# opherlieber/rltime

Measured on AMD Instinct MI355X. Metric: sampled transitions/sec (= learner steps/sec x B x T), IQN-LSTM B=512 T=80 84x84x4, higher is better.
Workload: dtype f32

## Files before the change

### include/mirl.h

```cpp
#ifndef MIRL_H
#define MIRL_H

#include <stdint.h>

#ifdef __cplusplus
extern "C" {
#endif

#define MIRL_OK 0
#define MIRL_NEED_MORE 1
#define MIRL_ERR_ARG (-1)
#define MIRL_ERR_HIP (-2)
#define MIRL_ERR_STATE (-3)
#define MIRL_ERR_NOGPU (-4)

#define MIRL_MODE_UNIFORM 0
#define MIRL_MODE_PER 1

typedef struct mirl_replay mirl_replay;

typedef struct mirl_replay_config {
  int64_t size;
  int32_t num_envs;
  int32_t env_base;
// ... 202 lines not shown
                              float* db, void* stream);

int mirl_conv1p3_u8_supported(int32_t H, int32_t W, int32_t F, int32_t K, int32_t S);
int mirl_conv1p3_u8_wpk_floats(int64_t* out);
int mirl_conv1p3_u8_fwd(int64_t N, int32_t H, int32_t W, const uint8_t* x, const float* weight,
                        int64_t ws_o, int64_t ws_c, int64_t ws_h, int64_t ws_w, const float* bias, float scale,
                        float* wpk, float* y, int32_t flags, void* stream);
int mirl_conv1p3_u8_wrw_scratch_floats(int64_t* out);
int mirl_conv1p3_u8_wrw(int64_t N, int32_t H, int32_t W, const uint8_t* x, const float* g, float scale,
                        float* scratch, float* dw, int64_t ws_o, int64_t ws_c, int64_t ws_h, int64_t ws_w, void* stream);
int mirl_conv1p3_u8_wrw_masked(int64_t N, int32_t H, int32_t W, const uint8_t* x, const float* dy, const float* y,
                               float scale, float* scratch, float* dw, int64_t ws_o, int64_t ws_c, int64_t ws_h,
                               int64_t ws_w, float* db, void* stream);

int mirl_conv2_bwd_data_supported(int32_t C, int32_t F, int32_t K, int32_t S, int32_t IH, int32_t IW,
                                  int32_t OH, int32_t OW);
int mirl_conv2_bwd_data(int64_t N, int32_t OH, int32_t OW, const float* g, const float* weight,
                        int64_t ws_o, int64_t ws_c, int64_t ws_h, int64_t ws_w, float* wpk, float* dx,
                        void* stream);
int mirl_conv2_bwd_data_wpk_floats(int64_t* floats);
int mirl_conv2_bwd_data_ex(int64_t N, int32_t OH, int32_t OW, const float* g, const float* weight, int64_t ws_o,
                           int64_t ws_c, int64_t ws_h, int64_t ws_w, float* wpk, int64_t wpk_floats, float* dx, int32_t pipe,
                           void* stream);
int mirl_conv3_bwd_data_supported(int32_t C, int32_t F, int32_t K, int32_t S, int32_t IH, int32_t IW, int32_t OH, int32_t OW);
int mirl_conv3_bwd_data_wpk_floats(int64_t* floats);
int mirl_conv3_bwd_data(int64_t N, int32_t OH, int32_t OW, const float* g, const float* weight, int64_t ws_o,
                        int64_t ws_c, int64_t ws_h, int64_t ws_w, float* wpk, int64_t wpk_floats, float* dx, void* stream);

int mirl_gemm3_supported(int32_t layout, int64_t M, int64_t N, int64_t K);
int mirl_gemm3_workspace_bytes(int32_t layout, int64_t M, int64_t N, int64_t K, int64_t* bytes);
int mirl_gemm3(int32_t layout, int64_t M, int64_t N, int64_t K, const float* A, int64_t lda,
               const float* B, int64_t ldb, float* C, int64_t ldc, const float* bias, int32_t relu,
               void* workspace, int64_t workspace_bytes, void* stream);
int mirl_gemm3_mid_set(int32_t mode);
int mirl_gemm3_nt_mul(int64_t M, int64_t N, int64_t K, const float* A, int64_t lda, const float* B,
                      int64_t ldb, float* C, int64_t ldc, const float* bias, int32_t relu,
                      const float* mul, int64_t ldmul, int32_t group_shift, float* pre, int64_t ldpre,
                      void* stream);
int mirl_gemm3_head_workspace_bytes(int64_t M, int64_t N, int64_t* bytes);
int mirl_gemm3_nt_head(int64_t M, int64_t N, int64_t K, const float* A, int64_t lda, const float* B, int64_t ldb,
                       float* C, int64_t ldc, const float* bias, int32_t relu, const float* w2, int32_t O,
                       const float* bias2, float* out2, int64_t ldo, void* workspace, int64_t workspace_bytes, void* stream);
int mirl_gemm3_nn_qp_partial_rows(int64_t M, int64_t* rows);
int mirl_gemm3_nn_qp(int64_t M, int64_t N, int64_t K, const float* A, int64_t lda, const float* B, int64_t ldb,
                     const float* emb, int64_t ldemb, const float* x, int64_t ldx, float* d_pre, int64_t ldd,
                     float* dx, int64_t lddx, float* db_partial, void* stream);

int mirl_conv3_fwd_supported(int32_t C, int32_t F, int32_t KH, int32_t KW, int32_t S, int32_t H, int32_t W);
int mirl_conv3_fwd(int64_t N, int32_t H, int32_t W, int32_t C, int32_t F, int32_t KH, int32_t KW, int32_t S,
                   const float* x, const float* w, const float* bias, int32_t relu, float* y, void* stream);

int mirl_conv_wrw_b3_supported(int32_t C, int32_t F, int32_t KH, int32_t KW, int32_t S, int32_t H, int32_t W);
int mirl_conv_wrw_b3_scratch_bytes(int32_t C, int32_t F, int32_t KH, int32_t KW, int64_t* bytes);
int mirl_conv_wrw_b3(int64_t N, int32_t H, int32_t W, int32_t C, int32_t F, int32_t KH, int32_t KW, int32_t S,
                     const float* x, const float* g, void* scratch, int64_t scratch_bytes, float* dw, void* stream);

int mirl_bias_relu_rows(int64_t rows, int32_t C, float* y, const float* bias, void* stream);
int mirl_colsum_blocks(int64_t rows, int32_t C, int32_t* blocks);
int mirl_relu_bwd_bias_rows(int64_t rows, int32_t C, const float* dy, const float* y, float* g,
                            float* db, float* partial, int32_t blocks, void* stream);
int mirl_cos_embed(int64_t rows, int32_t D, const float* tau, const float* freq, float* phi, void* stream);
int mirl_cos_embed_rng(int64_t rows, int32_t D, uint64_t seed, const uint64_t* step, const float* freq,
                       float* phi, float* tau_out, void* stream);
int mirl_iqn_mul_fwd(int64_t M, int32_t N, int32_t C, const float* x, const float* emb, float* out, void* stream);
int mirl_iqn_mul_bwd(int64_t M, int32_t N, int32_t C, const float* g, const float* emb, const float* x,
                     float* d_pre, float* dx, float* db, float* partial, int32_t blocks, void* stream);

int mirl_dueling_tail_bwd(int64_t M, int32_t H1, int32_t Hv, int32_t A, int32_t Q, const float* ga,
                          const float* gv, const float* wo, const float* wq, const float* both,
                          float* g, float* db, float* partial, int32_t blocks, void* stream);
int mirl_dueling_tail_bwd_w(int64_t M, int32_t H1, int32_t Hv, int32_t A, int32_t Q, const float* ga,
                            const float* gv, const float* wo, const float* wq, const float* both, float* g,
                            float* db, float* partial, int32_t blocks, float* dwj, float* partial_w,
                            void* stream);

int mirl_actor_head(int32_t E, int32_t N, int32_t A, const float* adv, const float* val, int32_t Q,
                    const double* eps, const double* expo, double eps_min, const float* u, const int64_t* rnd,
                    int32_t* actions, float* qvalues, float* eps_used, void* stream);
int mirl_actor_head_rng(int32_t E, int32_t N, int32_t A, const float* adv, int32_t adv_pitch, const float* val, int32_t Q,
                        const double* eps, const double* expo, double eps_min, uint64_t rng_seed,
                        const uint64_t* rng_step, int32_t* actions, float* qvalues, float* eps_used, void* stream);
int mirl_actor_head_c51(int32_t E, int32_t A, int32_t Z, const float* adv, int32_t adv_pitch, const float* val,
                        int32_t val_pitch, const float* support, const double* eps, const double* expo, double eps_min,
                        const float* u, const int64_t* rnd, uint64_t rng_seed, const uint64_t* rng_step,
                        int32_t* actions, float* qvalues, float* eps_used, void* stream);
int mirl_stack_shift(int32_t E, int32_t P, int32_t plane_bytes, const uint8_t* in, uint8_t* out,
                     const uint8_t* newest, const uint8_t* dones, void* stream);
#define MIRL_STEP_ADVANCE (~0ull)
int mirl_actor_pre(int32_t E, int32_t H, int32_t A, const float* rewards_raw, const uint8_t* dones,
                   const int32_t* actions, const float* h, const float* c, float* xh_tail, int64_t xh_pitch,
                   float* c_in, float* state_pack, float* initials, float* rewards_out, uint8_t* dones_out,
                   int32_t clip_rewards, float* ep_reward, int32_t* ep_len, float* out_reward, int32_t* out_len,
                   int32_t* action_counts, uint64_t* rng_step, uint64_t step, void* stream);
int mirl_synth_env_step(int32_t E, int64_t frame_bytes, const uint8_t* pool, int32_t pool_n, uint64_t* clock, int32_t slot,
                        uint64_t seed, float p_neg, float p_nonpos, float p_done, uint8_t* obs, float* rewards,
                        uint8_t* dones, void* stream);
int mirl_act_conv_supported(int32_t layer, int32_t Ci, int32_t Co, int32_t k, int32_t stride, int32_t Hi, int32_t Wi);
int mirl_act_conv_fwd(int32_t layer, int64_t frames, int32_t Hi, int32_t Wi, const float* x, const float* w_taps,
                      const float* bias, float* y, int64_t y_frame_pitch, void* stream);
int mirl_act_lstm_supported(int32_t E, int32_t H, int32_t K);
int mirl_act_lstm_workspace_bytes(int32_t E, int32_t H, int32_t K, int64_t* bytes);
int mirl_act_lstm_fwd(int32_t E, int32_t H, int32_t K, const float* xh, int64_t xh_pitch, const float* w, const float* bias,
                      const float* c_in, float* h_out, float* c_out, void* workspace, void* stream);
int mirl_act_embed(int32_t E, int32_t N, int32_t H, int32_t D, const float* h, const float* freq, const float* taus,
                   uint64_t seed, const uint64_t* step, const float* wq, const float* bq, float* x, float* tau_out, void* stream);
int mirl_act_head_supported(int32_t E, int32_t N, int32_t H, int32_t D, int32_t HID, int32_t NO);
// ... 153 lines not shown
```

### rltime_amd/_lib.py

```python
import ctypes as C
import os

import torch

_HERE = os.path.dirname(os.path.abspath(__file__))
LIB_PATH = os.path.join(_HERE, "librltime_hip.so")

MIRL_OK = 0
MIRL_NEED_MORE = 1
MODE_UNIFORM = 0
MODE_PER = 1
INT32_MIN = -2 ** 31


MIRL_OK, MIRL_ERR_ARG, MIRL_ERR_HIP, MIRL_ERR_STATE, MIRL_ERR_NOGPU = 0, -1, -2, -3, -4


class MirlError(RuntimeError):
    code = None


class ReplayConfig(C.Structure):
    _fields_ = [
        ("size", C.c_int64),
# ... 118 lines not shown
    "mirl_q_target_c51": [_i64, _i32, _i32, _vp, _vp, _vp, _vp, _vp, _vp, _f64, _f64, _f64, _f64, _i32, _vp, _vp],
    "mirl_loss_c51": [_i64, _i32, _i32, _vp, _vp, _vp, _vp, _i32, _f64, _f64, _vp, _vp, _vp, _vp],
    "mirl_actor_head_c51": [_i32, _i32, _i32, _vp, _i32, _vp, _i32, _vp, _vp, _vp, _f64, _vp, _vp, _u64, _vp, _vp, _vp, _vp, _vp],
    "mirl_lstm_cell_fwd": [_i32, _i32, _vp, _vp, _vp, _vp, _vp, _vp, _vp, _vp],
    "mirl_lstm_seq_supported": [_i32, _i32, _i32],
    "mirl_lstm_seq_workspace_bytes": [_i32, _i32, _P(_i64)],
    "mirl_lstm_seq_fwd": [_i32, _i32, _i32, _vp, _vp, _vp, _vp, _vp, _vp, _vp, _vp, _vp, _vp, _vp, _i32, _vp, _vp],
    "mirl_lstm_seq_status": [_P(_i32)],
    "mirl_gemm3_mid_set": [_i32],
    "mirl_lstm_seq_fwd_grid": [_i32, _i32, _P(_i32), _P(_i64), _P(_i32), _P(_i32)],
    "mirl_lstm_seq_bwd_supported": [_i32, _i32, _i32],
    "mirl_lstm_seq_bwd_workspace_bytes": [_i32, _i32, _P(_i64)],
    "mirl_lstm_seq_bwd": [_i32, _i32, _i32, _vp, _vp, _vp, _vp, _vp, _vp, _vp, _vp],
    "mirl_lstm_cell_bwd": [_i32, _i32, _vp, _vp, _vp, _vp, _vp, _vp, _vp, _i32, _vp],
    "mirl_lstm_extras_supported": [_i64, _i64, _i32],
    "mirl_lstm_extras_add": [_i64, _i64, _i32, _vp, _i64, _vp, _i64, _vp, _i64, _vp, _i64, _vp],
    "mirl_lstm_extras_wgrad_workspace_bytes": [_i64, _i64, _i32, _P(_i64)],
    "mirl_lstm_extras_wgrad": [_i64, _i64, _i32, _vp, _i64, _vp, _i64, _vp, _vp, _i64, _vp],
    "mirl_frames_to_f32_nhwc": [_i64, _i32, _i32, _vp, C.c_float, _vp, _vp],
    "mirl_frames_to_f32_nhwc_ex": [_i64, _i32, _i32, _vp, C.c_float, _vp, _i32, _i32, _vp],
    "mirl_conv1_u8_supported": [_i32, _i32, _i32, _i32, _i32, _i32],
    "mirl_conv1_bf16_set": [_i32],
    "mirl_conv1_wrw_bf16_set": [_i32],
    "mirl_conv1_u8_wpk_floats": [_P(_i64)],
    "mirl_conv1_u8_fwd": [_i64, _i32, _i32, _vp, _vp, _i64, _i64, _i64, _i64, _vp, C.c_float, _vp, _vp, _vp],
    "mirl_conv1_u8_fwd_ex": [_i64, _i32, _i32, _vp, _vp, _i64, _i64, _i64, _i64, _vp, C.c_float, _vp, _vp, _i32, _vp],
    "mirl_conv1_u8_wrw_scratch_floats": [_P(_i64)],
    "mirl_conv1_u8_wrw_ex": [_i64, _i32, _i32, _vp, _vp, C.c_float, _vp, _vp, _i64, _i64, _i64, _i64, _i32, _vp],
    "mirl_conv1_u8_wrw_masked": [_i64, _i32, _i32, _vp, _vp, _vp, C.c_float, _vp, _vp, _i64, _i64, _i64, _i64, _vp, _vp],
    "mirl_conv1_u8_wrw": [_i64, _i32, _i32, _vp, _vp, C.c_float, _vp, _vp, _i64, _i64, _i64, _i64, _vp],
    "mirl_conv1p_u8_supported": [_i32, _i32, _i32, _i32, _i32],
    "mirl_conv1p_u8_wpk_floats": [_P(_i64)],
    "mirl_conv1p_u8_fwd": [_i64, _i32, _i32, _vp, _vp, _i64, _i64, _i64, _vp, C.c_float, _vp, _vp, _i32, _vp],
    "mirl_conv1p_u8_wrw_scratch_floats": [_P(_i64)],
    "mirl_conv1p_u8_wrw": [_i64, _i32, _i32, _vp, _vp, C.c_float, _vp, _vp, _i64, _i64, _i64, _vp],
    "mirl_conv1p_u8_wrw_masked": [_i64, _i32, _i32, _vp, _vp, _vp, C.c_float, _vp, _vp, _i64, _i64, _i64, _vp, _vp],
    "mirl_conv1p3_u8_supported": [_i32, _i32, _i32, _i32, _i32],
    "mirl_conv1p3_u8_wpk_floats": [_P(_i64)],
    "mirl_conv1p3_u8_fwd": [_i64, _i32, _i32, _vp, _vp, _i64, _i64, _i64, _i64, _vp, C.c_float, _vp, _vp, _i32, _vp],
    "mirl_conv1p3_u8_wrw_scratch_floats": [_P(_i64)],
    "mirl_conv1p3_u8_wrw": [_i64, _i32, _i32, _vp, _vp, C.c_float, _vp, _vp, _i64, _i64, _i64, _i64, _vp],
    "mirl_conv1p3_u8_wrw_masked": [_i64, _i32, _i32, _vp, _vp, _vp, C.c_float, _vp, _vp, _i64, _i64, _i64, _i64, _vp, _vp],
    "mirl_conv2_bwd_data_supported": [_i32, _i32, _i32, _i32, _i32, _i32, _i32, _i32],
    "mirl_conv2_bwd_data": [_i64, _i32, _i32, _vp, _vp, _i64, _i64, _i64, _i64, _vp, _vp, _vp],
    "mirl_conv2_bwd_data_wpk_floats": [_P(_i64)],
    "mirl_conv3_bwd_data_supported": [_i32, _i32, _i32, _i32, _i32, _i32, _i32, _i32],
    "mirl_conv3_bwd_data_wpk_floats": [_P(_i64)],
    "mirl_conv3_bwd_data": [_i64, _i32, _i32, _vp, _vp, _i64, _i64, _i64, _i64, _vp, _i64, _vp, _vp],
    "mirl_conv2_bwd_data_ex": [_i64, _i32, _i32, _vp, _vp, _i64, _i64, _i64, _i64, _vp, _i64, _vp, _i32, _vp],
    "mirl_conv3_fwd_supported": [_i32, _i32, _i32, _i32, _i32, _i32, _i32],
    "mirl_conv3_fwd": [_i64, _i32, _i32, _i32, _i32, _i32, _i32, _i32, _vp, _vp, _vp, _i32, _vp, _vp],
    "mirl_conv_wrw_b3_supported": [_i32, _i32, _i32, _i32, _i32, _i32, _i32],
    "mirl_conv_wrw_b3_scratch_bytes": [_i32, _i32, _i32, _i32, _P(_i64)],
    "mirl_conv_wrw_b3": [_i64, _i32, _i32, _i32, _i32, _i32, _i32, _i32, _vp, _vp, _vp, _i64, _vp, _vp],
    "mirl_gemm3_supported": [_i32, _i64, _i64, _i64],
    "mirl_gemm3_workspace_bytes": [_i32, _i64, _i64, _i64, _P(_i64)],
    "mirl_gemm3": [_i32, _i64, _i64, _i64, _vp, _i64, _vp, _i64, _vp, _i64, _vp, _i32, _vp, _i64, _vp],
    "mirl_gemm3_nt_mul": [_i64, _i64, _i64, _vp, _i64, _vp, _i64, _vp, _i64, _vp, _i32, _vp, _i64, _i32, _vp, _i64, _vp],
    "mirl_gemm3_nn_qp_partial_rows": [_i64, _P(_i64)],
    "mirl_gemm3_nn_qp": [_i64, _i64, _i64, _vp, _i64, _vp, _i64, _vp, _i64, _vp, _i64, _vp, _i64, _vp, _i64, _vp, _vp],
    "mirl_gemm3_head_workspace_bytes": [_i64, _i64, _P(_i64)],
    "mirl_gemm3_nt_head": [_i64, _i64, _i64, _vp, _i64, _vp, _i64, _vp, _i64, _vp, _i32, _vp, _i32, _vp, _vp, _i64, _vp, _i64, _vp],
    "mirl_act_conv_supported": [_i32, _i32, _i32, _i32, _i32, _i32, _i32],
    "mirl_act_conv_fwd": [_i32, _i64, _i32, _i32, _vp, _vp, _vp, _vp, _i64, _vp],
    "mirl_act_lstm_supported": [_i32, _i32, _i32],
    "mirl_act_lstm_workspace_bytes": [_i32, _i32, _i32, _P(_i64)],
    "mirl_act_lstm_fwd": [_i32, _i32, _i32, _vp, _i64, _vp, _vp, _vp, _vp, _vp, _vp, _vp],
    "mirl_act_embed": [_i32, _i32, _i32, _i32, _vp, _vp, _vp, _u64, _vp, _vp, _vp, _vp, _vp, _vp],
    "mirl_act_head_supported": [_i32, _i32, _i32, _i32, _i32, _i32],
    "mirl_act_head_parts": [_i32, _i32, _P(_i32), _P(_i32)],
    "mirl_act_head_hidden": [_i32, _i32, _i32, _i32, _vp, _vp, _vp, _vp, _vp, _vp],
    "mirl_act_head_select": [_i32, _i32, _i32, _i32, _i32, _vp, _vp, _i32, _vp, _vp, _f64, _u64, _vp, _vp, _vp, _vp],
    "mirl_bias_relu_rows": [_i64, _i32, _vp, _vp, _vp],
    "mirl_colsum_blocks": [_i64, _i32, _P(_i32)],
    "mirl_relu_bwd_bias_rows": [_i64, _i32, _vp, _vp, _vp, _vp, _vp, _i32, _vp],
    "mirl_cos_embed": [_i64, _i32, _vp, _vp, _vp, _vp],
    "mirl_cos_embed_rng": [_i64, _i32, _u64, _vp, _vp, _vp, _vp, _vp],
    "mirl_adam_clip_workspace_bytes": [_i32, _vp, _vp],
    "mirl_adam_clip_step": [_i32, _vp, _vp, _vp, _vp, _vp, _vp, _f64, _vp, _f64, _f64, _f64, _f64, _vp, _i64, _vp, _vp],
    "mirl_adam_clip_step_guarded": [_i32, _vp, _vp, _vp, _vp, _vp, _vp, _f64, _vp, _f64, _f64, _f64, _f64, _vp, _i64, _vp, _vp, _vp],
    "mirl_step_guard_open": [_vp, _vp, _i64, _vp, _i32, _vp],
    "mirl_replay_update_losses_guarded": [_vp, _i64, _vp, _vp, _vp, _vp],
    "mirl_lstm_seq_status_device": [_P(_vp)],
    "mirl_iqn_mul_fwd": [_i64, _i32, _i32, _vp, _vp, _vp, _vp],
    "mirl_iqn_mul_bwd": [_i64, _i32, _i32, _vp, _vp, _vp, _vp, _vp, _vp, _vp, _i32, _vp],
    "mirl_dueling_tail_bwd": [_i64, _i32, _i32, _i32, _i32, _vp, _vp, _vp, _vp, _vp, _vp, _vp, _vp, _i32, _vp],
    "mirl_dueling_tail_bwd_w": [_i64, _i32, _i32, _i32, _i32, _vp, _vp, _vp, _vp, _vp, _vp, _vp, _vp, _i32, _vp, _vp, _vp],
    "mirl_actor_head": [_i32, _i32, _i32, _vp, _vp, _i32, _vp, _vp, _f64, _vp, _vp, _vp, _vp, _vp, _vp],
    "mirl_actor_head_rng": [_i32, _i32, _i32, _vp, _i32, _vp, _i32, _vp, _vp, _f64, _u64, _vp, _vp, _vp, _vp, _vp],
    "mirl_actor_head_ac": [_i32, _i32, _vp, _i64, _vp, _vp, _i32, _vp, _vp, _vp, _i32, _vp],
    "mirl_actor_head_ac_rng": [_i32, _i32, _vp, _i64, _vp, _i64, _u64, _vp, _i32, _vp, _vp, _vp, _i32, _vp],
    "mirl_online_append": [_i32, _i32, _vp, _i32, _i64, _vp, _vp, _vp, _vp, _vp, _i64, _i32, _vp, _vp, _vp, _vp, _vp, _vp, _vp, _vp,
                           _vp, _vp],
    "mirl_online_advance": [_vp, _i64, _vp],
    "mirl_online_window": [_i32, _i32, _i32, _i32, _i32, _f64, _f64, _i64, _vp, _vp, _vp, _vp, _vp, _vp, _vp, _i32, _vp, _vp, _vp, _vp,
                           _vp, _vp, _vp, _vp, _vp],
    "mirl_ac_loss": [_i64, _i32, _vp, _i64, _vp, _vp, _vp, _vp, _vp, _f64, _f64, _f64, _i32, _vp, _i64, _vp, _vp, _vp, _vp],
    "mirl_actor_head_normal": [_i32, _i32, _vp, _i64, _vp, _vp, _vp, _vp, _vp, _vp, _i32, _vp],
    "mirl_online_window_box": [_i32, _i32, _i32, _i32, _i32, _f64, _f64, _i64, _vp, _vp, _vp, _vp, _vp, _vp, _vp, _i32, _vp, _vp, _vp,
                               _vp, _vp, _vp, _vp, _vp, _i32, _vp],
    "mirl_online_window_rec": [_i32, _i32, _i32, _i32, _i32, _f64, _f64, _i64, _vp, _vp, _vp, _vp, _vp, _vp, _vp, _i32, _vp, _vp, _vp,
                               _vp, _vp, _vp, _vp, _vp, _i32, _vp, _vp, _i32, _vp, _vp, _vp, _vp, _vp],
    "mirl_ac_loss_normal": [_i64, _i32, _vp, _i64, _vp, _vp, _vp, _vp, _vp, _vp, _f64, _f64, _f64, _i32, _vp, _i64, _vp, _vp, _vp, _vp,
                            _vp],
    "mirl_stack_shift": [_i32, _i32, _i32, _vp, _vp, _vp, _vp, _vp],
    "mirl_synth_env_step": [_i32, _i64, _vp, _i32, _vp, _i32, _u64, C.c_float, C.c_float, C.c_float, _vp, _vp, _vp, _vp],
# ... 96 lines not shown
```

### rltime_amd/csrc/conv_wrw.hip

```cpp
#include "common.hpp"
#include "split3.hpp"
#include <stdlib.h>

namespace mirl {

typedef float cw_f4 __attribute__((ext_vector_type(4)));

constexpr int CW_F = 64;
constexpr int CW_MAXT = 5;

struct CwArgs {
  const float* x; const float* g; float* partial;
  int N, H, W, C, KH, KW, S, OH, OW;
  int T;
  int NT;
  int FPI;
  int KP;
  int Cp;
  int xplane;
  int gpitch;
};

template <int TPW>
__global__ void __launch_bounds__(512) __attribute__((amdgpu_waves_per_eu(2, 2)))
k_conv_wrw_b3(CwArgs a) {
  extern __shared__ __align__(16) char cw_lds[];
  uint16_t* xs = reinterpret_cast<uint16_t*>(cw_lds);
  uint16_t* gs = xs + 3 * a.xplane;
  int* tbl = reinterpret_cast<int*>(gs + 3 * CW_F * a.gpitch);
  const int tid = threadIdx.x, lane = tid & 63, wave = __builtin_amdgcn_readfirstlane(tid >> 6);
  const int j = lane & 15, kq = lane >> 4;
  const int OHW = a.OH * a.OW, fx = a.H * a.W * a.C, gplane = CW_F * a.gpitch;
  const int ksteps = a.KP >> 5;
  for (int p = tid; p < a.KP; p += 512) {
    const int f = p / OHW, r = p - f * OHW, oh = r / a.OW, ow = r - oh * a.OW;
    tbl[p] = f < a.FPI ? ((f * a.H + a.S * oh) * a.W + a.S * ow) * a.Cp : 0;
  }
  for (int o = tid; o < 3 * a.xplane / 8; o += 512) reinterpret_cast<uint4*>(xs)[o] = make_uint4(0u, 0u, 0u, 0u);
  const int nt0 = wave * TPW;
  int toff[TPW];
#pragma unroll
  for (int i = 0; i < TPW; ++i) {
    int t = (nt0 + i) * 16 + j; if (t > a.T - 1) t = a.T - 1;
    const int c = t % a.C, kk = t / a.C, kw = kk % a.KW, kh = kk / a.KW;
    toff[i] = (kh * a.W + kw) * a.Cp + c;
  }
  g3_f32x4 acc[4][TPW];
#pragma unroll
  for (int m = 0; m < 4; ++m)
#pragma unroll
    for (int i = 0; i < TPW; ++i) acc[m][i] = g3_f32x4{0.f, 0.f, 0.f, 0.f};

  const int units = (a.N + a.FPI - 1) / a.FPI;
  auto put_x = [&](const cw_f4& v, int o) {
    const float q[4] = {v.x, v.y, v.z, v.w};
    uint2 h, m, l;
    g3_split4(q, h, m, l);
    const int pix = (o * 4) / a.C, c0 = o * 4 - pix * a.C;
    uint32_t* d = reinterpret_cast<uint32_t*>(xs + pix * a.Cp + c0);
    d[0] = h.x; d[1] = h.y;
    d[a.xplane / 2] = m.x; d[a.xplane / 2 + 1] = m.y;
    d[a.xplane] = l.x; d[a.xplane + 1] = l.y;
  };
  auto load_g8 = [&](float (&q)[8], const float* gu, int item, int valid_pos) {
    const int f = item & 63, p0 = (item >> 6) * 8;
#pragma unroll
    for (int e = 0; e < 8; ++e) {
      const int p = p0 + e;
      const float t = gu[(int64_t)(p < valid_pos ? p : valid_pos - 1) * CW_F + f];
      q[e] = p < valid_pos ? t : 0.f;
    }
  };
  auto put_g8 = [&](const float (&q)[8], int item) {
    const int f = item & 63, p0 = (item >> 6) * 8;
    const float q0[4] = {q[0], q[1], q[2], q[3]}, q1[4] = {q[4], q[5], q[6], q[7]};
    uint2 h0, m0, l0, h1, m1, l1;
    g3_split4(q0, h0, m0, l0);
    g3_split4(q1, h1, m1, l1);
// ... 45 lines not shown
        for (int p = 0; p < 3; ++p)
#pragma unroll
          for (int e = 0; e < 8; ++e) r[p][e] = xs[p * a.xplane + org[e] + toff[i]];
      };
      read_b(raw[0], 0);
#pragma unroll
      for (int i = 0; i < TPW; ++i) {
        if (i + 1 < TPW) read_b(raw[(i + 1) & 1], i + 1);
        __builtin_amdgcn_sched_barrier(0);
        g3_bf16x8 bf[3];
#pragma unroll
        for (int p = 0; p < 3; ++p) {
          const uint32_t* r = raw[i & 1][p];
          bf[p] = __builtin_bit_cast(g3_bf16x8, make_uint4(r[0] | (r[1] << 16), r[2] | (r[3] << 16), r[4] | (r[5] << 16), r[6] | (r[7] << 16)));
        }
        constexpr int PA[6] = {2, 0, 1, 1, 0, 0};
        constexpr int PB[6] = {0, 2, 1, 0, 1, 0};
#pragma unroll
        for (int c = 0; c < 6; ++c)
#pragma unroll
          for (int m = 0; m < 4; ++m)
            acc[m][i] = __builtin_amdgcn_mfma_f32_16x16x32_bf16(af[m][PA[c]], bf[PB[c]], acc[m][i], 0, 0, 0);
        __builtin_amdgcn_sched_barrier(0);
      }
    }
  }
  float* out = a.partial + (int64_t)blockIdx.x * CW_F * a.T;
#pragma unroll
  for (int i = 0; i < TPW; ++i) {
    const int t = (nt0 + i) * 16 + j;
    if (nt0 + i < a.NT) {
#pragma unroll
      for (int m = 0; m < 4; ++m)
#pragma unroll
        for (int r = 0; r < 4; ++r) out[(int64_t)(16 * m + 4 * kq + r) * a.T + t] = acc[m][i][r];
    }
  }
}

__global__ void __launch_bounds__(256)
k_conv_wrw_reduce(const cw_f4* __restrict__ partial, int parts, int64_t n4, cw_f4* __restrict__ dw) {
  const int64_t i = (int64_t)blockIdx.x * 256 + threadIdx.x;
  if (i >= n4) return;
  cw_f4 s0 = {0.f, 0.f, 0.f, 0.f}, s1 = s0, s2 = s0, s3 = s0;
  int p = 0;
  for (; p + 4 <= parts; p += 4) {
    s0 += partial[(int64_t)p * n4 + i]; s1 += partial[(int64_t)(p + 1) * n4 + i];
    s2 += partial[(int64_t)(p + 2) * n4 + i]; s3 += partial[(int64_t)(p + 3) * n4 + i];
  }
  for (; p < parts; ++p) s0 += partial[(int64_t)p * n4 + i];
  dw[i] = (s0 + s1) + (s2 + s3);
}

static int cw_geometry(int64_t N, int H, int W, int C, int F, int KH, int KW, int S, CwArgs* a, size_t* lds, unsigned* grid) {
  if (F != CW_F || C < 4 || (C % 4) || KH < 1 || KW < 1 || S < 1 || H < KH || W < KW) return 0;
  const int T = KH * KW * C;
  if (T % 16) return 0;
  const int NT = T / 16;
  if (NT > 8 * CW_MAXT) return 0;
  const int OH = (H - KH) / S + 1, OW = (W - KW) / S + 1, OHW = OH * OW;
  if ((OHW * CW_F) % 4) return 0;
  int best = 0;
  size_t best_lds = 0;
  double best_waste = 0.0;
  for (int fpi = 1; fpi <= 4; ++fpi) {
    const int KP = (fpi * OHW + 31) / 32 * 32;
    const int xplane = (fpi * H * W * (C + 2) + 7) / 8 * 8;
    const size_t need = (size_t)3 * xplane * 2 + (size_t)3 * CW_F * (KP + 8) * 2 + (size_t)KP * 4;
    if (need > 150 * 1024) break;
    const double waste = (double)KP / (fpi * OHW);
    if (!best || waste <= best_waste + 1e-9) { best = fpi; best_lds = need; best_waste = waste; }
  }
  if (!best) return 0;
  if (a) {
    a->N = (int)N; a->H = H; a->W = W; a->C = C; a->KH = KH; a->KW = KW; a->S = S; a->OH = OH; a->OW = OW;
    a->T = T; a->NT = NT; a->FPI = best; a->KP = (best * OHW + 31) / 32 * 32;
    a->Cp = C + 2; a->xplane = (best * H * W * (C + 2) + 7) / 8 * 8; a->gpitch = a->KP + 8;
    const int64_t units = (N + best - 1) / best;
    *grid = capped_grid(units, 256);
    *lds = best_lds;
  }
  return 1;
}

}

extern "C" int mirl_conv_wrw_b3_supported(int32_t C, int32_t F, int32_t KH, int32_t KW, int32_t S, int32_t H, int32_t W) {
  return mirl::cw_geometry(1, H, W, C, F, KH, KW, S, nullptr, nullptr, nullptr);
}

extern "C" int mirl_conv_wrw_b3_scratch_bytes(int32_t C, int32_t F, int32_t KH, int32_t KW, int64_t* bytes) {
  if (!bytes || F != mirl::CW_F || C < 1 || KH < 1 || KW < 1) return mirl::fail(MIRL_ERR_ARG, "conv_wrw_b3_scratch_bytes: bad arguments");
  *bytes = (int64_t)256 * F * KH * KW * C * (int64_t)sizeof(float);
  return MIRL_OK;
}

extern "C" int mirl_conv_wrw_b3(int64_t N, int32_t H, int32_t W, int32_t C, int32_t F, int32_t KH, int32_t KW, int32_t S,
                                const float* x, const float* g, void* scratch, int64_t scratch_bytes, float* dw, void* stream) {
  using namespace mirl;
  CwArgs a;
  size_t lds = 0;
  unsigned grid = 0;
  if (N <= 0 || N >= (1LL << 30) || !x || !g || !scratch || !dw) return fail(MIRL_ERR_ARG, "bad conv_wrw_b3 arguments");
  if (!cw_geometry(N, H, W, C, F, KH, KW, S, &a, &lds, &grid)) return fail(MIRL_ERR_ARG, "conv_wrw_b3: unsupported layer shape");
  if (!aligned16(x, g, scratch, dw)) return fail(MIRL_ERR_ARG, "conv_wrw_b3: pointers must be 16-byte aligned");
  if (scratch_bytes < (int64_t)grid * CW_F * a.T * (int64_t)sizeof(float)) return fail(MIRL_ERR_ARG, "conv_wrw_b3: scratch too small");
  a.x = x; a.g = g; a.partial = (float*)scratch;
  hipStream_t st = (hipStream_t)stream;
  const int tpw = (a.NT + 7) / 8;
  const void* fns[CW_MAXT] = {(const void*)k_conv_wrw_b3<1>, (const void*)k_conv_wrw_b3<2>, (const void*)k_conv_wrw_b3<3>,
                              (const void*)k_conv_wrw_b3<4>, (const void*)k_conv_wrw_b3<5>};
  const void* fn = fns[tpw - 1];
  if (int rc = raise_lds_limit(fn, 150 * 1024)) return rc;
  {
    ProfScope ps("k_conv_wrw_b3", 4.0 * (double)N * ((double)H * W * C + (double)a.OH * a.OW * CW_F), st,
                 2.0 * (double)N * a.OH * a.OW * CW_F * a.T);
    void* kargs[] = {(void*)&a};
    MIRL_HIP(hipLaunchKernel(fn, dim3(grid), dim3(512), kargs, lds, st));
  }
  ProfScope ps("k_conv_wrw_reduce", (double)(grid + 1) * CW_F * a.T * 4.0, st);
  const int64_t n4 = (int64_t)CW_F * a.T / 4;
  hipLaunchKernelGGL(k_conv_wrw_reduce, dim3((unsigned)((n4 + 255) / 256)), dim3(256), 0, st, reinterpret_cast<const cw_f4*>(scratch),
                     (int)grid, n4, reinterpret_cast<cw_f4*>(dw));
  MIRL_LAUNCH_CHECK();
  return MIRL_OK;
}
```

### rltime_amd/csrc/host_util.hpp

```cpp
#pragma once
#include <stddef.h>
#include <stdint.h>

namespace mirl {

inline unsigned magic_u32(int64_t d) { return d > 1 ? (unsigned)(((1ULL << 32) + (uint64_t)d - 1) / (uint64_t)d) : 0u; }

template <typename... P>
inline bool aligned16(const P*... p) { return ((((uintptr_t)p % 16) == 0) && ...); }

inline unsigned capped_grid(int64_t units, int64_t cap) { return (unsigned)(units < cap ? units : cap); }

constexpr int C1_PLANES = 4, C1_K = 8, C1_S = 4, C1_F = 32, C1_TAPS = C1_K * C1_K;
constexpr int C1_DW = C1_F * C1_PLANES * C1_TAPS;
constexpr int C1_WGS = 512;
constexpr int C1_WPK_FLOATS = 3 * 2 * C1_K * 64 * 4;
constexpr int C1_WLO_BYTES = 2 * C1_K * 64 * 16;
constexpr size_t C1_LDS = 64 * 1024, C1_LDS_WRW_B3 = 80 * 1024, C1_LDS_FWD_BF = 96 * 1024;
constexpr int C1P_DW = C1_F * C1_TAPS;
constexpr int C1P_SLAB = C1P_DW + C1_F;
constexpr int C1P_WGS = 1024;
constexpr int C1P_FWD_WGS = 1024;
constexpr int C1P_FPI = 4;
constexpr int C1P_WPK = 3 * 2 * 2 * 64 * 4;
// ... 36 lines not shown
inline C1FwdPlan c1_fwd_plan(int64_t N, int H, int W, bool bf, int fpi, int split) {
  const int pitch = c1_pitch(H * W), tiles = (c1_out(H) * c1_out(W) + 15) / 16;
  const bool fits2 = (size_t)2 * C1_PLANES * pitch <= C1_LDS;
  if (fpi != 1 && fpi != 2) fpi = (N >= 1024 && fits2) ? 2 : 1;
  if (fpi == 2 && !fits2) fpi = 1;
  const int max_split = (tiles + 3) / 4;
  if (split <= 0) split = N >= C1_WGS ? 1 : (int)((C1_WGS + N - 1) / N);
  if (split > max_split) split = max_split;
  if (fpi == 2) split = 1;
  return {fpi, split, capped_grid((N + fpi - 1) / fpi * split, C1_WGS), (size_t)fpi * C1_PLANES * pitch + (bf ? C1_WLO_BYTES : 0)};
}
inline C1FwdPlan c1p_fwd_plan(int64_t N, int H, int W) {
  const int HW = H * W, tiles = (c1_out(H) * c1_out(W) + 15) / 16;
  int fpi_max = 32 * 1024 / HW;
  fpi_max = fpi_max < 1 ? 1 : (fpi_max > C1P_FPI ? C1P_FPI : fpi_max);
  const int64_t fpi64 = N / C1P_FWD_WGS;
  const int fpi = fpi64 < 1 ? 1 : (fpi64 > fpi_max ? fpi_max : (int)fpi64);
  const int max_split = (tiles + 3) / 4;
  int split = N >= C1P_FWD_WGS ? 1 : (int)((C1P_FWD_WGS + N - 1) / N);
  if (split > max_split) split = max_split;
  return {fpi, split, capped_grid((N + fpi - 1) / fpi * split, C1P_FWD_WGS), (size_t)fpi * HW};
}

inline C1FwdPlan c3p_fwd_plan(int64_t N, int H, int W) {
  const int HW3 = C3P_PLANES * H * W, tiles = (c1_out(H) * c1_out(W) + 15) / 16;
  int fpi_max = C3P_FILL / HW3;
  fpi_max = fpi_max < 1 ? 1 : (fpi_max > C3P_FPI ? C3P_FPI : fpi_max);
  const int64_t fpi64 = N / C3P_WGS;
  const int fpi = fpi64 < 1 ? 1 : (fpi64 > fpi_max ? fpi_max : (int)fpi64);
  const int max_split = (tiles + 3) / 4;
  int split = N >= C3P_WGS ? 1 : (int)((C3P_WGS + N - 1) / N);
  if (split > max_split) split = max_split;
  return {fpi, split, capped_grid((N + fpi - 1) / fpi * split, C3P_WGS), (size_t)fpi * HW3};
}

struct C1WrwPlan { bool bf16; int fpi, pitch, slab; unsigned grid; size_t lds; };
inline size_t c1_at_least_slab(size_t lds, int slab) { return lds < (size_t)slab * 4 ? (size_t)slab * 4 : lds; }
inline C1WrwPlan c1_wrw_plan(int64_t N, int H, int W, bool masked, bool allow_bf16) {
  const int HW = H * W, slab = C1_DW + (masked ? C1_F : 0), Pd = c1_bf_pitch(HW, c1_out(W)), pitch = c1_pitch(HW);
  if (allow_bf16 && (size_t)C1_PLANES * Pd * 2 <= C1_LDS_WRW_B3)
    return {true, 1, Pd, slab, capped_grid(N, C1_WGS), c1_at_least_slab((size_t)C1_PLANES * Pd * 2, slab)};
  const int fpi = (N >= 1024 && (size_t)2 * C1_PLANES * pitch <= C1_LDS) ? 2 : 1;
  return {false, fpi, pitch, slab, capped_grid((N + fpi - 1) / fpi, C1_WGS), c1_at_least_slab((size_t)fpi * C1_PLANES * pitch, slab)};
}
inline C1WrwPlan c1p_wrw_plan(int64_t N, int H, int W) {
  const int Pd = c1_bf_pitch(H * W, c1_out(W));
  return {true, 1, Pd, C1P_SLAB, capped_grid(N, C1P_WGS), c1_at_least_slab((size_t)Pd * 2, C1P_SLAB)};
}
inline C1WrwPlan c3p_wrw_plan(int64_t N, int H, int W) {
  const int Pd = c1_bf_pitch(H * W, c1_out(W));
  return {true, 1, Pd, C3P_SLAB, capped_grid(N, C3P_WGS), c1_at_least_slab((size_t)C3P_PLANES * Pd * 2, C3P_SLAB)};
}

}
```

Baseline: 481,400.

## Stream conv weight-gradient inputs through an LDS row ring with software pipelining

```diff
diff --git a/include/mirl.h b/include/mirl.h
--- a/include/mirl.h
+++ b/include/mirl.h
@@ -278,6 +278,7 @@
 
 int mirl_conv_wrw_b3_supported(int32_t C, int32_t F, int32_t KH, int32_t KW, int32_t S, int32_t H, int32_t W);
 int mirl_conv_wrw_b3_scratch_bytes(int32_t C, int32_t F, int32_t KH, int32_t KW, int64_t* bytes);
+int mirl_conv_wrw_b3_plan(int64_t N, int32_t C, int32_t F, int32_t KH, int32_t KW, int32_t S, int32_t H, int32_t W, int32_t* out);
 int mirl_conv_wrw_b3(int64_t N, int32_t H, int32_t W, int32_t C, int32_t F, int32_t KH, int32_t KW, int32_t S,
                      const float* x, const float* g, void* scratch, int64_t scratch_bytes, float* dw, void* stream);
 
diff --git a/rltime_amd/_lib.py b/rltime_amd/_lib.py
--- a/rltime_amd/_lib.py
+++ b/rltime_amd/_lib.py
@@ -194,6 +194,7 @@
     "mirl_conv3_fwd": [_i64, _i32, _i32, _i32, _i32, _i32, _i32, _i32, _vp, _vp, _vp, _i32, _vp, _vp],
     "mirl_conv_wrw_b3_supported": [_i32, _i32, _i32, _i32, _i32, _i32, _i32],
     "mirl_conv_wrw_b3_scratch_bytes": [_i32, _i32, _i32, _i32, _P(_i64)],
+    "mirl_conv_wrw_b3_plan": [_i64, _i32, _i32, _i32, _i32, _i32, _i32, _i32, _P(_i32)],
     "mirl_conv_wrw_b3": [_i64, _i32, _i32, _i32, _i32, _i32, _i32, _i32, _vp, _vp, _vp, _i64, _vp, _vp],
     "mirl_gemm3_supported": [_i32, _i64, _i64, _i64],
     "mirl_gemm3_workspace_bytes": [_i32, _i64, _i64, _i64, _P(_i64)],
diff --git a/rltime_amd/csrc/conv_wrw.hip b/rltime_amd/csrc/conv_wrw.hip
--- a/rltime_amd/csrc/conv_wrw.hip
+++ b/rltime_amd/csrc/conv_wrw.hip
@@ -2,14 +2,224 @@
 #include "split3.hpp"
 #include <stdlib.h>
 
+#ifndef CW_PF
+#define CW_PF 2
+#endif
+
 namespace mirl {
 
 typedef float cw_f4 __attribute__((ext_vector_type(4)));
-
-constexpr int CW_F = 64;
-constexpr int CW_MAXT = 5;
+typedef unsigned short cw_u16x8 __attribute__((ext_vector_type(8)));
 
 struct CwArgs {
+  const float* x; const float* g; float* partial;
+  int64_t N;
+  int H, W, C, KH, KW, S, OH, OW;
+  int T;
+  int NT;
+  int Cp;
+  int rowhw;
+  int xplane;
+  int ring;
+  int rowv, cq;
+  unsigned m_ohw, m_ow, m_rowv, m_cq;
+};
+
+template <int LX>
+struct CwStage {
+  cw_f4 v[LX];
+  float q[8];
+  const cw_f4* src;
+  int rows, slot;
+  int valid;
+};
+
+template <int TPW, int LX>
+__global__ void __launch_bounds__(512) __attribute__((amdgpu_waves_per_eu(2, 2)))
+k_conv_wrw_b3(CwArgs a) {
+  static_assert(CW_PF == 2 || CW_PF == 3, "stages in flight");
+  constexpr int NS = CW_PF - 1;
+  constexpr int gplane = CW_F * CW_GPITCH;
+  extern __shared__ __align__(16) char cw_lds[];
+  uint16_t* xs = reinterpret_cast<uint16_t*>(cw_lds);
+  uint16_t* gs = xs + 3 * a.xplane;
+  int* tbl = reinterpret_cast<int*>(gs + CW_G_HALFWORDS);
+  const int tid = threadIdx.x, lane = tid & 63, wave = __builtin_amdgcn_readfirstlane(tid >> 6);
+  const int j = lane & 15, kq = lane >> 4;
+  const int OHW = a.OH * a.OW;
+  int64_t n0;
+  int frames;
+  cw_frames(a.N, gridDim.x, blockIdx.x, &n0, &frames);
+  const int64_t P = (int64_t)frames * OHW;
+  const int ksteps = (int)((P + CW_KS - 1) / CW_KS);
+  const int nt0 = wave * TPW;
+  int toff[TPW];
+#pragma unroll
+  for (int i = 0; i < TPW; ++i) {
+    int t = (nt0 + i) * 16 + j; if (t > a.T - 1) t = a.T - 1;
+    const int c = t % a.C, kk = t / a.C, kw = kk % a.KW, kh = kk / a.KW;
+    toff[i] = (kh * a.W + kw) * a.Cp + c;
+  }
+  g3_f32x4 acc[4][TPW];
+#pragma unroll
+  for (int m = 0; m < 4; ++m)
+#pragma unroll
+    for (int i = 0; i < TPW; ++i) acc[m][i] = g3_f32x4{0.f, 0.f, 0.f, 0.f};
+
+  CwPos last = {0, -1};
+  int front_f = 0, front_end = 0, fslot = 0;
+  const cw_f4* xsrc = reinterpret_cast<const cw_f4*>(a.x + n0 * ((int64_t)a.H * a.W * a.C));
+  const float* gsrc = a.g + n0 * ((int64_t)OHW * CW_F);
+  int64_t left = P;
+  const int gf = tid & 63, gp0 = ((tid >> 6) & 3) * 8;
+  auto load = [&](CwStage<LX>& s) {
+    const CwPos b = cw_step(last, CW_KS, OHW, a.m_ohw, frames);
+    const int end = cw_row_end(b, a.m_ow, a.S, a.KH);
+    s.rows = (b.f - front_f) * a.H + end - front_end;
+    s.slot = fslot;
+    s.src = xsrc;
+    const int nv = s.rows * a.rowv;
+#pragma unroll
+    for (int k = 0; k < LX; ++k) {
+      const int o = tid + k * 512;
+      s.v[k] = cw_f4{0.f, 0.f, 0.f, 0.f};
+      if (o < nv) s.v[k] = xsrc[o];
+    }
+    xsrc += nv;
+    fslot += s.rows;
+    if (fslot >= a.ring) fslot -= a.ring;
+    front_f = b.f; front_end = end; last = b;
+    s.valid = left < CW_KS ? (left > 0 ? (int)left : 0) : CW_KS;
+    left -= CW_KS;
+#pragma unroll
+    for (int e = 0; e < 8; ++e) {
+      s.q[e] = 0.f;
+      if (tid >= 256 && gp0 + e < s.valid) s.q[e] = gsrc[(gp0 + e) * CW_F + gf];
+    }
+    gsrc += CW_KS * CW_F;
+  };
+  auto put_x = [&](const cw_f4& v, int o, int slot0) {
+    const float q[4] = {v.x, v.y, v.z, v.w};
+    uint2 h, m, l;
+    g3_split4(q, h, m, l);
+    const unsigned ri = cw_div((unsigned)o, a.m_rowv), rem = (unsigned)o - ri * a.rowv, pix = cw_div(rem, a.m_cq), c0 = (rem - pix * a.cq) * 4;
+    int slot = slot0 + (int)ri;
+    if (slot >= a.ring) slot -= a.ring;
+    uint32_t* d = reinterpret_cast<uint32_t*>(xs + slot * a.rowhw + pix * a.Cp + c0);
+    d[0] = h.x; d[1] = h.y;
+    d[a.xplane / 2] = m.x; d[a.xplane / 2 + 1] = m.y;
+    d[a.xplane] = l.x; d[a.xplane + 1] = l.y;
+    if (slot < a.KH - 1) {
+      d += a.ring * a.rowhw / 2;
+      d[0] = h.x; d[1] = h.y;
+      d[a.xplane / 2] = m.x; d[a.xplane / 2 + 1] = m.y;
+      d[a.xplane] = l.x; d[a.xplane + 1] = l.y;
+    }
+  };
+  CwPos tpos = {0, 0};
+  int tslot = 0;
+  auto store = [&](const CwStage<LX>& s, int buf) {
+    const int nv = s.rows * a.rowv;
+#pragma unroll
+    for (int k = 0; k < LX; ++k) { const int o = tid + k * 512; if (o < nv) put_x(s.v[k], o, s.slot); }
+    for (int o = tid + LX * 512; o < nv; o += 512) put_x(s.src[o], o, s.slot);
+    if (s.valid <= 0) return;
+    if (tid >= 256) {
+      const float q0[4] = {s.q[0], s.q[1], s.q[2], s.q[3]}, q1[4] = {s.q[4], s.q[5], s.q[6], s.q[7]};
+      uint2 h0, m0, l0, h1, m1, l1;
+      g3_split4(q0, h0, m0, l0);
+      g3_split4(q1, h1, m1, l1);
+      uint16_t* d = gs + buf * 3 * gplane + gf * CW_GPITCH + gp0;
+      *reinterpret_cast<uint4*>(d) = make_uint4(h0.x, h0.y, h1.x, h1.y);
+      *reinterpret_cast<uint4*>(d + gplane) = make_uint4(m0.x, m0.y, m1.x, m1.y);
+      *reinterpret_cast<uint4*>(d + 2 * gplane) = make_uint4(l0.x, l0.y, l1.x, l1.y);
+    }
+    if (wave == 0) {
+      const unsigned r = (unsigned)(tpos.r + (lane & 31));
+      unsigned q = cw_div(r, a.m_ohw);
+      unsigned rr = r - q * (unsigned)OHW;
+      if (tpos.f + (int)q >= frames) { q = (unsigned)(frames - 1 - tpos.f); rr = (unsigned)(OHW - 1); }
+      const unsigned oh = cw_div(rr, a.m_ow), ow = rr - oh * (unsigned)a.OW;
+      const unsigned slot = ((unsigned)tslot + q * (unsigned)a.H + (unsigned)a.S * oh) % (unsigned)a.ring;
+      if (lane < 32) tbl[buf * CW_KS + lane] = (int)((slot * (unsigned)a.W + (unsigned)a.S * ow) * (unsigned)a.Cp);
+      const unsigned r0 = (unsigned)(tpos.r + CW_KS), q0 = cw_div(r0, a.m_ohw);
+      tpos.f += (int)q0;
+      tpos.r = (int)(r0 - q0 * (unsigned)OHW);
+      tslot = (int)(((unsigned)tslot + q0 * (unsigned)a.H) % (unsigned)a.ring);
+    }
+  };
+  auto multiply = [&](int buf) {
+    const uint16_t* gb = gs + buf * 3 * gplane;
+    int org[8];
+    {
+      const int4 t0 = *reinterpret_cast<const int4*>(tbl + buf * CW_KS + kq * 8), t1 = *reinterpret_cast<const int4*>(tbl + buf * CW_KS + kq * 8 + 4);
+      org[0] = t0.x; org[1] = t0.y; org[2] = t0.z; org[3] = t0.w; org[4] = t1.x; org[5] = t1.y; org[6] = t1.z; org[7] = t1.w;
+    }
+    g3_bf16x8 af[4][3];
+#pragma unroll
+    for (int m = 0; m < 4; ++m)
+#pragma unroll
+      for (int p = 0; p < 3; ++p)
+        af[m][p] = *reinterpret_cast<const g3_bf16x8*>(gb + p * gplane + (16 * m + j) * CW_GPITCH + kq * 8);
+    cw_u16x8 raw[2][3];
+    auto read_b = [&](cw_u16x8 (&r)[3], int i) {
+#pragma unroll
+      for (int p = 0; p < 3; ++p)
+#pragma unroll
+        for (int e = 0; e < 8; ++e) r[p][e] = xs[p * a.xplane + org[e] + toff[i]];
+    };
+    read_b(raw[0], 0);
+#pragma unroll
+    for (int i = 0; i < TPW; ++i) {
+      if (i + 1 < TPW) read_b(raw[(i + 1) & 1], i + 1);
+      __builtin_amdgcn_sched_barrier(0);
+      g3_bf16x8 bf[3];
+#pragma unroll
+      for (int p = 0; p < 3; ++p) bf[p] = __builtin_bit_cast(g3_bf16x8, raw[i & 1][p]);
+      constexpr int PA[6] = {2, 0, 1, 1, 0, 0};
+      constexpr int PB[6] = {0, 2, 1, 0, 1, 0};
+#pragma unroll
+      for (int c = 0; c < 6; ++c)
+#pragma unroll
+        for (int m = 0; m < 4; ++m)
+          acc[m][i] = __builtin_amdgcn_mfma_f32_16x16x32_bf16(af[m][PA[c]], bf[PB[c]], acc[m][i], 0, 0, 0);
+      __builtin_amdgcn_sched_barrier(0);
+    }
+  };
+
+  CwStage<LX> st[NS];
+  load(st[0]);
+  store(st[0], 0);
+#pragma unroll
+  for (int u = 1; u < CW_PF; ++u) load(st[u % NS]);
+  g3_barrier();
+  for (int k0 = 0; k0 < ksteps; k0 += NS) {
+#pragma unroll
+    for (int u = 0; u < NS; ++u) {
+      const int k = k0 + u;
+      if (k < ksteps) {
+        CwStage<LX>& s = st[(u + 1) % NS];
+        store(s, (k + 1) & 1);
+        load(s);
+        multiply(k & 1);
+        g3_barrier();
+      }
+    }
+  }
+  float* out = a.partial + (int64_t)blockIdx.x * CW_F * a.T;
+#pragma unroll
+  for (int i = 0; i < TPW; ++i) {
+    const int t = (nt0 + i) * 16 + j;
+    if (nt0 + i < a.NT) {
+#pragma unroll
+      for (int m = 0; m < 4; ++m)
+#pragma unroll
+        for (int r = 0; r < 4; ++r) out[(int64_t)(16 * m + 4 * kq + r) * a.T + t] = acc[m][i][r];
+    }
+  }
+}
+
+struct CwFramesArgs {
   const float* x; const float* g; float* partial;
   int N, H, W, C, KH, KW, S, OH, OW;
   int T;
@@ -23,7 +233,7 @@
 
 template <int TPW>
 __global__ void __launch_bounds__(512) __attribute__((amdgpu_waves_per_eu(2, 2)))
-k_conv_wrw_b3(CwArgs a) {
+k_conv_wrw_b3_frames(CwFramesArgs a) {
   extern __shared__ __align__(16) char cw_lds[];
   uint16_t* xs = reinterpret_cast<uint16_t*>(cw_lds);
   uint16_t* gs = xs + 3 * a.xplane;
@@ -175,76 +385,74 @@
   dw[i] = (s0 + s1) + (s2 + s3);
 }
 
-static int cw_geometry(int64_t N, int H, int W, int C, int F, int KH, int KW, int S, CwArgs* a, size_t* lds, unsigned* grid) {
-  if (F != CW_F || C < 4 || (C % 4) || KH < 1 || KW < 1 || S < 1 || H < KH || W < KW) return 0;
-  const int T = KH * KW * C;
-  if (T % 16) return 0;
-  const int NT = T / 16;
-  if (NT > 8 * CW_MAXT) return 0;
-  const int OH = (H - KH) / S + 1, OW = (W - KW) / S + 1, OHW = OH * OW;
-  if ((OHW * CW_F) % 4) return 0;
-  int best = 0;
-  size_t best_lds = 0;
-  double best_waste = 0.0;
-  for (int fpi = 1; fpi <= 4; ++fpi) {
-    const int KP = (fpi * OHW + 31) / 32 * 32;
-    const int xplane = (fpi * H * W * (C + 2) + 7) / 8 * 8;
-    const size_t need = (size_t)3 * xplane * 2 + (size_t)3 * CW_F * (KP + 8) * 2 + (size_t)KP * 4;
-    if (need > 150 * 1024) break;
-    const double waste = (double)KP / (fpi * OHW);
-    if (!best || waste <= best_waste + 1e-9) { best = fpi; best_lds = need; best_waste = waste; }
-  }
-  if (!best) return 0;
-  if (a) {
-    a->N = (int)N; a->H = H; a->W = W; a->C = C; a->KH = KH; a->KW = KW; a->S = S; a->OH = OH; a->OW = OW;
-    a->T = T; a->NT = NT; a->FPI = best; a->KP = (best * OHW + 31) / 32 * 32;
-    a->Cp = C + 2; a->xplane = (best * H * W * (C + 2) + 7) / 8 * 8; a->gpitch = a->KP + 8;
-    const int64_t units = (N + best - 1) / best;
-    *grid = capped_grid(units, 256);
-    *lds = best_lds;
-  }
-  return 1;
+template <int TPW>
+static const void* cw_stream_fn(int lx) {
+  return lx <= 2 ? (const void*)k_conv_wrw_b3<TPW, 2> : (const void*)k_conv_wrw_b3<TPW, 4>;
 }
 
 }
 
 extern "C" int mirl_conv_wrw_b3_supported(int32_t C, int32_t F, int32_t KH, int32_t KW, int32_t S, int32_t H, int32_t W) {
-  return mirl::cw_geometry(1, H, W, C, F, KH, KW, S, nullptr, nullptr, nullptr);
+  return mirl::cw_shape_ok(C, F, KH, KW, S, H, W) ? 1 : 0;
 }
 
 extern "C" int mirl_conv_wrw_b3_scratch_bytes(int32_t C, int32_t F, int32_t KH, int32_t KW, int64_t* bytes) {
   if (!bytes || F != mirl::CW_F || C < 1 || KH < 1 || KW < 1) return mirl::fail(MIRL_ERR_ARG, "conv_wrw_b3_scratch_bytes: bad arguments");
-  *bytes = (int64_t)256 * F * KH * KW * C * (int64_t)sizeof(float);
+  *bytes = mirl::cw_scratch_bytes(C, KH, KW);
+  return MIRL_OK;
+}
+
+extern "C" int mirl_conv_wrw_b3_plan(int64_t N, int32_t C, int32_t F, int32_t KH, int32_t KW, int32_t S, int32_t H, int32_t W, int32_t* out) {
+  using namespace mirl;
+  if (!out || N <= 0 || N >= (1LL << 30) || !cw_shape_ok(C, F, KH, KW, S, H, W)) return fail(MIRL_ERR_ARG, "conv_wrw_b3_plan: bad arguments");
+  const CwPlan p = cw_plan(N, C, KH, KW, S, H, W);
+  out[0] = p.stream ? 1 : 0; out[1] = p.ring; out[2] = p.enter; out[3] = (int32_t)p.lds; out[4] = (int32_t)p.grid; out[5] = p.fpi;
   return MIRL_OK;
 }
 
 extern "C" int mirl_conv_wrw_b3(int64_t N, int32_t H, int32_t W, int32_t C, int32_t F, int32_t KH, int32_t KW, int32_t S,
                                 const float* x, const float* g, void* scratch, int64_t scratch_bytes, float* dw, void* stream) {
   using namespace mirl;
-  CwArgs a;
-  size_t lds = 0;
-  unsigned grid = 0;
   if (N <= 0 || N >= (1LL << 30) || !x || !g || !scratch || !dw) return fail(MIRL_ERR_ARG, "bad conv_wrw_b3 arguments");
-  if (!cw_geometry(N, H, W, C, F, KH, KW, S, &a, &lds, &grid)) return fail(MIRL_ERR_ARG, "conv_wrw_b3: unsupported layer shape");
+  if (!cw_shape_ok(C, F, KH, KW, S, H, W)) return fail(MIRL_ERR_ARG, "conv_wrw_b3: unsupported layer shape");
   if (!aligned16(x, g, scratch, dw)) return fail(MIRL_ERR_ARG, "conv_wrw_b3: pointers must be 16-byte aligned");
-  if (scratch_bytes < (int64_t)grid * CW_F * a.T * (int64_t)sizeof(float)) return fail(MIRL_ERR_ARG, "conv_wrw_b3: scratch too small");
-  a.x = x; a.g = g; a.partial = (float*)scratch;
+  const CwPlan p = cw_plan(N, C, KH, KW, S, H, W);
+  if (scratch_bytes < (int64_t)p.grid * CW_F * p.T * (int64_t)sizeof(float)) return fail(MIRL_ERR_ARG, "conv_wrw_b3: scratch too small");
   hipStream_t st = (hipStream_t)stream;
-  const int tpw = (a.NT + 7) / 8;
-  const void* fns[CW_MAXT] = {(const void*)k_conv_wrw_b3<1>, (const void*)k_conv_wrw_b3<2>, (const void*)k_conv_wrw_b3<3>,
-                              (const void*)k_conv_wrw_b3<4>, (const void*)k_conv_wrw_b3<5>};
-  const void* fn = fns[tpw - 1];
-  if (int rc = raise_lds_limit(fn, 150 * 1024)) return rc;
+  const int tpw = (p.NT + 7) / 8;
   {
-    ProfScope ps("k_conv_wrw_b3", 4.0 * (double)N * ((double)H * W * C + (double)a.OH * a.OW * CW_F), st,
-                 2.0 * (double)N * a.OH * a.OW * CW_F * a.T);
-    void* kargs[] = {(void*)&a};
-    MIRL_HIP(hipLaunchKernel(fn, dim3(grid), dim3(512), kargs, lds, st));
-  }
-  ProfScope ps("k_conv_wrw_reduce", (double)(grid + 1) * CW_F * a.T * 4.0, st);
-  const int64_t n4 = (int64_t)CW_F * a.T / 4;
+    const double bytes = 4.0 * (double)N * ((double)H * W * C + (double)p.OH * p.OW * CW_F), flops = 2.0 * (double)N * p.OH * p.OW * CW_F * p.T;
+    if (p.stream) {
+      CwArgs a;
+      a.x = x; a.g = g; a.partial = (float*)scratch; a.N = N;
+      a.H = H; a.W = W; a.C = C; a.KH = KH; a.KW = KW; a.S = S; a.OH = p.OH; a.OW = p.OW; a.T = p.T; a.NT = p.NT;
+      a.Cp = C + 2; a.rowhw = p.rowhw; a.xplane = p.xplane; a.ring = p.ring; a.rowv = W * C / 4; a.cq = C / 4;
+      a.m_ohw = magic_u32(p.OH * p.OW); a.m_ow = magic_u32(p.OW); a.m_rowv = magic_u32(a.rowv); a.m_cq = magic_u32(a.cq);
+      const int lx = (p.enter * a.rowv + 511) / 512;
+      const void* fns[CW_MAXT] = {cw_stream_fn<1>(lx), cw_stream_fn<2>(lx), cw_stream_fn<3>(lx), cw_stream_fn<4>(lx), cw_stream_fn<5>(lx)};
+      const void* fn = fns[tpw - 1];
+      if (int rc = raise_lds_limit(fn, (int)CW_LDS)) return rc;
+      ProfScope ps("k_conv_wrw_b3", bytes, st, flops);
+      void* kargs[] = {(void*)&a};
+      MIRL_HIP(hipLaunchKernel(fn, dim3(p.grid), dim3(512), kargs, p.lds, st));
+    } else {
+      CwFramesArgs a;
+      a.x = x; a.g = g; a.partial = (float*)scratch; a.N = (int)N;
+      a.H = H; a.W = W; a.C = C; a.KH = KH; a.KW = KW; a.S = S; a.OH = p.OH; a.OW = p.OW; a.T = p.T; a.NT = p.NT;
+      a.FPI = p.fpi; a.KP = p.KP; a.Cp = C + 2; a.xplane = p.xplane; a.gpitch = p.gpitch;
+      const void* fns[CW_MAXT] = {(const void*)k_conv_wrw_b3_frames<1>, (const void*)k_conv_wrw_b3_frames<2>, (const void*)k_conv_wrw_b3_frames<3>,
+                                  (const void*)k_conv_wrw_b3_frames<4>, (const void*)k_conv_wrw_b3_frames<5>};
+      const void* fn = fns[tpw - 1];
+      if (int rc = raise_lds_limit(fn, (int)CW_LDS)) return rc;
+      ProfScope ps("k_conv_wrw_b3", bytes, st, flops);
+      void* kargs[] = {(void*)&a};
+      MIRL_HIP(hipLaunchKernel(fn, dim3(p.grid), dim3(512), kargs, p.lds, st));
+    }
+  }
+  ProfScope ps("k_conv_wrw_reduce", (double)(p.grid + 1) * CW_F * p.T * 4.0, st);
+  const int64_t n4 = (int64_t)CW_F * p.T / 4;
   hipLaunchKernelGGL(k_conv_wrw_reduce, dim3((unsigned)((n4 + 255) / 256)), dim3(256), 0, st, reinterpret_cast<const cw_f4*>(scratch),
-                     (int)grid, n4, reinterpret_cast<cw_f4*>(dw));
+                     (int)p.grid, n4, reinterpret_cast<cw_f4*>(dw));
   MIRL_LAUNCH_CHECK();
   return MIRL_OK;
 }
diff --git a/rltime_amd/csrc/host_util.hpp b/rltime_amd/csrc/host_util.hpp
--- a/rltime_amd/csrc/host_util.hpp
+++ b/rltime_amd/csrc/host_util.hpp
@@ -112,4 +112,101 @@
   return {true, 1, Pd, C3P_SLAB, capped_grid(N, C3P_WGS), c1_at_least_slab((size_t)C3P_PLANES * Pd * 2, C3P_SLAB)};
 }
 
-}
+#if defined(__HIPCC__)
+#define MIRL_HD __host__ __device__
+#else
+#define MIRL_HD
+#endif
+constexpr int CW_F = 64;
+constexpr int CW_MAXT = 5;
+constexpr int CW_WGS = 256;
+constexpr int CW_KS = 32;
+constexpr int CW_GPITCH = CW_KS + 8;
+constexpr int CW_G_HALFWORDS = 2 * 3 * CW_F * CW_GPITCH;
+constexpr size_t CW_LDS = 150 * 1024;
+
+MIRL_HD inline unsigned cw_div(unsigned n, unsigned magic) { return magic ? (unsigned)(((uint64_t)n * magic) >> 32) : n; }
+
+struct CwPos { int f, r; };
+MIRL_HD inline CwPos cw_step(CwPos p, int by, int OHW, unsigned m_ohw, int frames) {
+  const unsigned r = (unsigned)(p.r + by), q = cw_div(r, m_ohw);
+  p.f += (int)q;
+  p.r = (int)(r - q * (unsigned)OHW);
+  if (p.f >= frames) { p.f = frames - 1; p.r = OHW - 1; }
+  return p;
+}
+MIRL_HD inline int cw_row0(CwPos p, unsigned m_ow, int S) { return S * (int)cw_div((unsigned)p.r, m_ow); }
+MIRL_HD inline int cw_row_end(CwPos p, unsigned m_ow, int S, int KH) { return cw_row0(p, m_ow, S) + KH; }
+MIRL_HD inline void cw_frames(int64_t N, unsigned grid, unsigned b, int64_t* n0, int* frames) {
+  const int64_t q = N / grid, rem = N % grid;
+  *n0 = b * q + ((int64_t)b < rem ? (int64_t)b : rem);
+  *frames = (int)(q + ((int64_t)b < rem ? 1 : 0));
+}
+
+inline bool cw_shape_ok(int C, int F, int KH, int KW, int S, int H, int W) {
+  if (F != CW_F || C < 4 || (C % 4) || KH < 1 || KW < 1 || S < 1 || H < KH || W < KW) return false;
+  if ((int64_t)KH * KW * C > 16 * 8 * CW_MAXT || (KH * KW * C) % 16) return false;
+  if ((int64_t)H * W * (C + 2) > (int64_t)CW_LDS) return false;
+  const int OHW = ((H - KH) / S + 1) * ((W - KW) / S + 1), KP = (OHW + 31) / 32 * 32, xplane = (H * W * (C + 2) + 7) / 8 * 8;
+  return (size_t)3 * xplane * 2 + (size_t)3 * CW_F * (KP + 8) * 2 + (size_t)KP * 4 <= CW_LDS;
+}
+
+struct CwPlan {
+  bool stream;
+  int OH, OW, T, NT;
+  int ring, enter;
+  int rowhw;
+  int xplane;
+  int fpi, KP, gpitch;
+  size_t lds;
+  unsigned grid;
+};
+
+inline void cw_ring_need(int H, int OH, int OW, int S, int KH, int* ring, int* enter) {
+  const int OHW = OH * OW, frames = 1 << 30;
+  const unsigned m_ohw = magic_u32(OHW), m_ow = magic_u32(OW);
+  CwPos first = {0, 0}, last = cw_step(CwPos{0, -1}, CW_KS, OHW, m_ohw, frames);
+  int64_t F0 = (int64_t)last.f * H + cw_row_end(last, m_ow, S, KH);
+  int64_t need = F0, most = F0;
+  for (int k = 0; k <= OHW + 1; ++k) {
+    const CwPos next = cw_step(last, CW_KS, OHW, m_ohw, frames);
+    const int64_t F1 = (int64_t)next.f * H + cw_row_end(next, m_ow, S, KH), lo = (int64_t)first.f * H + cw_row0(first, m_ow, S);
+    if (F1 - F0 > most) most = F1 - F0;
+    if (F1 - lo > need) need = F1 - lo;
+    first = cw_step(first, CW_KS, OHW, m_ohw, frames);
+    last = next;
+    F0 = F1;
+  }
+  *ring = (int)need;
+  *enter = (int)most;
+}
+
+inline CwPlan cw_plan(int64_t N, int C, int KH, int KW, int S, int H, int W) {
+  CwPlan p = {};
+  p.OH = (H - KH) / S + 1; p.OW = (W - KW) / S + 1; p.T = KH * KW * C; p.NT = p.T / 16;
+  p.rowhw = W * (C + 2);
+  const int OHW = p.OH * p.OW;
+  cw_ring_need(H, p.OH, p.OW, S, KH, &p.ring, &p.enter);
+  const int64_t xplane = ((int64_t)(p.ring + KH - 1) * p.rowhw + 7) / 8 * 8;
+  const int64_t lds = 3 * xplane * 2 + (int64_t)CW_G_HALFWORDS * 2 + 2 * CW_KS * 4;
+  if (lds <= (int64_t)CW_LDS && (int64_t)p.enter * W * C / 4 < 65536 && OHW + CW_KS < 65536) {
+    p.stream = true;
+    p.xplane = (int)xplane; p.gpitch = CW_GPITCH; p.lds = (size_t)lds;
+    p.grid = capped_grid(N, CW_WGS);
+    return p;
+  }
+  double best_waste = 0.0;
+  for (int fpi = 1; fpi <= 4; ++fpi) {
+    const int KP = (fpi * OHW + 31) / 32 * 32, xp = (fpi * H * W * (C + 2) + 7) / 8 * 8;
+    const size_t need = (size_t)3 * xp * 2 + (size_t)3 * CW_F * (KP + 8) * 2 + (size_t)KP * 4;
+    if (need > CW_LDS) break;
+    const double waste = (double)KP / (fpi * OHW);
+    if (!p.fpi || waste <= best_waste + 1e-9) { p.fpi = fpi; p.KP = KP; p.xplane = xp; p.lds = need; best_waste = waste; }
+  }
+  p.gpitch = p.KP + 8;
+  p.grid = capped_grid((N + p.fpi - 1) / p.fpi, CW_WGS);
+  return p;
+}
+inline int64_t cw_scratch_bytes(int C, int KH, int KW) { return (int64_t)CW_WGS * CW_F * KH * KW * C * (int64_t)sizeof(float); }
+
+}
```

Result: no change. 483,900, median of 6 (+0.5%).
